# sarphiv/nerf-experiments

Measured on AMD Instinct MI355X. Metric: ray-samples/sec (coarse+fine), training step, higher is better.
Workload: dtype fp32

## Files before the change

### nerf-experiments_amd/csrc/mlp_fused.hip

```cpp
#include <stddef.h>
#include <stdlib.h>
#include <string.h>

#include <type_traits>

#include "common.h"
#include "encode_common.h"
#include "composite_common.h"
#include "hashgrid_common.h"

using namespace nerf;

typedef float f4 __attribute__((ext_vector_type(4)));
typedef float f8 __attribute__((ext_vector_type(8)));
typedef __bf16 bf16x8 __attribute__((ext_vector_type(8)));
typedef __bf16 bf16x4 __attribute__((ext_vector_type(4)));

namespace {

typedef __attribute__((address_space(3))) void lds_void_t;
typedef __attribute__((address_space(1))) void glb_void_t;

constexpr int SLOT_BYTES = 16 * 1024;
constexpr int NSLOT = 2;
// ... 223 lines not shown
template <int NS, class CT>
__device__ __forceinline__ void gen_hash_rows(const CT& c, int base, const float (&v)[9]) {
#pragma clang fp contract(off)
    float* R = reinterpret_cast<float*>(c.ximg);
    float* P = R + NS * GEN_LD;
    const int L = HG(int32_t, levels), F = HG(int32_t, features), T = HG(int32_t, table_size);
    const int cols = L * F;
    if (c.lane < NS) {
        float p[3] = {0.f, 0.f, 0.f};
        if (base + c.lane < c.M) {
            const float tq = HG(int32_t, query) == 0 ? v[6] : (v[6] + v[7]) / 2.0f;
            p[0] = v[0] + tq * v[3];
            p[1] = v[1] + tq * v[4];
            p[2] = v[2] + tq * v[5];
        }
        float* pr = P + c.lane * 8;
        pr[0] = p[0]; pr[1] = p[1]; pr[2] = p[2];
        float* row = R + c.lane * GEN_LD;
        for (int col = cols; col < 64; ++col) row[col] = 0.f;
    }
    const int normalize = HG(int32_t, normalize);
    const __attribute__((address_space(4))) int64_t* primes =
        (const __attribute__((address_space(4))) int64_t*)(c.kargs + offsetof(FusedArgs, hg) +
                                                           offsetof(nerf_hashgrid_params, primes));
    const long long pr[3] = {(long long)primes[0], (long long)primes[1], (long long)primes[2]};
    const __attribute__((address_space(4))) int32_t* res =
        (const __attribute__((address_space(4))) int32_t*)(c.kargs + offsetof(FusedArgs, hg) +
                                                           offsetof(nerf_hashgrid_params, res));
    const __attribute__((address_space(4))) int* offs =
        (const __attribute__((address_space(4))) int*)(c.kargs + offsetof(FusedArgs, hg_off));
    const float* table = *(const __attribute__((address_space(4))) cfptr_t*)(c.kargs + offsetof(FusedArgs, hg_table));
    for (int l = 0; l < L; ++l) {
        const int rl = res[l], ol = offs[l];
        if (c.lane < NS) {
            const int r = c.lane;
            const float p[3] = {P[r * 8 + 0], P[r * 8 + 1], P[r * 8 + 2]};
            const Corners cn = level_corners(p, normalize, rl, T, pr);
            const float* tab = table + (int64_t)ol * F;
            float* o = R + r * GEN_LD + l * F;
            float g[8][4];
#pragma unroll
            for (int k = 0; k < 8; ++k)
#pragma unroll
                for (int f = 0; f < 4; ++f) g[k][f] = f < F ? tab[(int64_t)cn.idx[k] * F + f] : 0.f;
            float acc[4] = {0.0f, 0.0f, 0.0f, 0.0f};
#pragma unroll
            for (int k = 0; k < 8; ++k)
#pragma unroll
                for (int f = 0; f < 4; ++f) acc[f] = acc[f] + cn.w[k] * g[k][f];
#pragma unroll
            for (int f = 0; f < 4; ++f)
                if (f < F) o[f] = acc[f];
        }
    }
}

template <int NS, class CT>
__device__ __forceinline__ void gen_rows_lds(const CT& c, int e, int base, const float (&v)[9]) {
#pragma clang fp contract(off)
    float* R = reinterpret_cast<float*>(c.ximg);
    float* P = R + NS * GEN_LD;
    const __attribute__((address_space(4))) nerf_pe_params& prm = EF(nerf_pe_params, params, e);
    if (prm.kind == 2) {
        gen_hash_rows<NS>(c, base, v);
        return;
    }
    const int per_ray = EF(int, per_ray, e);
    const int out_dim = EF(int, out_dim, e);
    const int L = prm.levels, id = prm.include_identity ? 3 : 0;
    if (c.lane < NS) {
        float pm[3] = {0.f, 0.f, 0.f}, vb[3] = {0.f, 0.f, 0.f};
        if (base + c.lane < c.M) {
            float p[3], dv[3];
            if (per_ray) {
                p[0] = v[0]; p[1] = v[1]; p[2] = v[2];
                dv[0] = dv[1] = dv[2] = 0.f;
            } else {
                const float tq = prm.query == 0 ? v[6] : (v[6] + v[7]) / 2.0f;
                dv[0] = v[3]; dv[1] = v[4]; dv[2] = v[5];
                p[0] = v[0] + tq * dv[0];
                p[1] = v[1] + tq * dv[1];
                p[2] = v[2] + tq * dv[2];
            }
            if (prm.kind == 1) {
                const IpeSample q = ipe_sample(prm, p, dv, v[6], v[7], v[8]);
                pm[0] = q.pm[0]; pm[1] = q.pm[1]; pm[2] = q.pm[2];
                vb[0] = q.vb[0]; vb[1] = q.vb[1]; vb[2] = q.vb[2];
            } else {
                pm[0] = p[0]; pm[1] = p[1]; pm[2] = p[2];
            }
        }
        float* pr = P + c.lane * 8;
        pr[0] = pm[0]; pr[1] = pm[1]; pr[2] = pm[2];
        pr[3] = vb[0]; pr[4] = vb[1]; pr[5] = vb[2];
        float* row = R + c.lane * GEN_LD;
        for (int col = 0; col < id; ++col) row[col] = pm[col];
        for (int col = out_dim; col < 64; ++col) row[col] = 0.f;
    }
    const int na = 3 * L;
    {
        static_assert(NS >= 16 && NS <= 64 && 64 % NS == 0, "mask lanes 0-15 in the g = 0 group");
        constexpr int G = 64 / NS;
        const int r = c.lane % NS, g = c.lane / NS;
        const float* pr = P + r * 8;
        const float pmr[3] = {pr[0], pr[1], pr[2]}, vbr[3] = {pr[3], pr[4], pr[5]};
        const float mreg = prm.use_mask ? prm.mask[c.lane & 15] : 1.f;
        const float scale = prm.scale;
        const int kind = prm.kind, use_mask = prm.use_mask;
        float* row = R + r * GEN_LD + id;
        for (int j = g; j < na; j += G) {
            const int dd = j >= 2 * L ? 2 : (j >= L ? 1 : 0);
            const int k = j - dd * L;
            const float sc = scale * (float)(1u << k);
            float sn, cs;
            sincos_enc(sel3(pmr, dd) * sc, &sn, &cs);
            if (kind == 1) {
                const float w = expf((-(sel3(vbr, dd) * (float)(1u << (2 * k)))) / 2.0f);
                cs = cs * w;
                sn = sn * w;
            }
            if (use_mask) {
                const float mk = __builtin_bit_cast(float, __builtin_amdgcn_ds_bpermute(k << 2, __builtin_bit_cast(int, mreg)));
                cs = mk * cs;
                sn = mk * sn;
            }
            row[j] = cs;
            row[na + j] = sn;
        }
    }
}

template <int NS, class CT>
__device__ __forceinline__ void gen_store(const CT& c, int e, int base) {
    const float* R = reinterpret_cast<const float*>(c.ximg);
    float* out = EF(fptr_t, out, e);
    const int per_ray = EF(int, per_ray, e);
    const unsigned S = (unsigned)EF(int, samples_per_ray, e);
    const int ld = (int)EF(int64_t, ld, e);
    const int q4 = ld >> 2;
    for (int i = c.lane; i < NS * q4; i += 64) {
        const int r = i / q4, q = i - r * q4;
        const int m = base + r;
        if (m < c.M && (!per_ray || (unsigned)m % S == 0u)) {
            const int64_t n = per_ray ? (int64_t)((unsigned)m / S) : (int64_t)m;
            *reinterpret_cast<f4*>(out + n * ld + 4 * q) = *reinterpret_cast<const f4*>(R + r * GEN_LD + 4 * q);
        }
    }
}

template <class CT>
__device__ __forceinline__ void gen_block(const CT& c, int r, int col, bf16x8& h, bf16x8& lo) {
    const float* R = reinterpret_cast<const float*>(c.ximg) + r * GEN_LD + col;
    const f4 v0 = *reinterpret_cast<const f4*>(R), v1 = *reinterpret_cast<const f4*>(R + 4);
    split8(__builtin_shufflevector(v0, v1, 0, 1, 2, 3, 4, 5, 6, 7), h, lo);
}

__device__ __forceinline__ void comp_grad_block(const Ctx& c, int gen, const float* coef, const int (&sample)[SB],
                                                const bool (&row_ok)[SB], bf16x8 (&h)[SB], bf16x8 (&lo)[SB]) {
#pragma clang fp contract(off)
    const unsigned S = (unsigned)CF(int32_t, samples_per_ray);
    const float* grgb = CF(cfptr_t, grad_rgb);
    const bool dens_head = CF(int32_t, sigma_layer) < 0;
    float* out = gen == 3 ? CF(fptr_t, grad_head) : CF(fptr_t, grad_sigma);
    const int64_t ldo = gen == 3 ? CF(int64_t, ld_head) : CF(int64_t, ld_sigma);
#pragma unroll
    for (int sb = 0; sb < SB; ++sb) {
        f4 x0 = {0.f, 0.f, 0.f, 0.f};
        if ((c.lane >> 4) == 0 && row_ok[sb]) {
            const unsigned m = (unsigned)sample[sb];
            const unsigned ray = m / S;
            const f4 q0 = *reinterpret_cast<const f4*>(coef + (size_t)m * 8);
            const f4 q1 = *reinterpret_cast<const f4*>(coef + (size_t)m * 8 + 4);
            const float g0 = grgb[ray * 3 + 0], g1 = grgb[ray * 3 + 1], g2 = grgb[ray * 3 + 2];
            const float ds = (g0 * q1[0] + g1 * q1[1]) + g2 * q1[2];
            if (gen == 3)
                x0 = f4{g0 * q0[0], g1 * q0[1], g2 * q0[2], dens_head ? ds : 0.f};
            else
                x0 = f4{ds, 0.f, 0.f, 0.f};
            if (out != nullptr) __builtin_nontemporal_store(x0, reinterpret_cast<f4*>(out + (size_t)m * ldo));
        }
        split8(__builtin_shufflevector(x0, f4{0.f, 0.f, 0.f, 0.f}, 0, 1, 2, 3, 4, 5, 6, 7), h[sb], lo[sb]);
    }
}

struct LayerState {
    int floor_i;
    bool qsplit;
    int col_chunk;
    int n1;
    unsigned bias_off;
    unsigned row_off[SB];
    unsigned row_off2[SB];
    int colok, colok2;
    unsigned sample_off[SB];
    unsigned mrow_off[SB];
    __amdgpu_buffer_rsrc_t ro, rm, rc, ro2;
    unsigned mw[SB][2];
    f4 stash[SB];
    unsigned pa[SB], pb[SB];
    unsigned pa2[SB], pb2[SB];
    int last_even;
    unsigned mi[SB][2];
    unsigned mcur[SB];
};

__device__ __forceinline__ void split2(float x, float y, unsigned& hi, unsigned& lo) {
    typedef __bf16 bf16x2 __attribute__((ext_vector_type(2)));
    typedef float f2 __attribute__((ext_vector_type(2)));
    const bf16x2 h = __builtin_convertvector((f4{x, y, 0.f, 0.f}).xy, bf16x2);
    hi = __builtin_bit_cast(unsigned, h);
    const f2 hf = {__builtin_bit_cast(float, hi << 16), __builtin_bit_cast(float, hi & 0xffff0000u)};
    const f2 d = f2{x, y} - hf;
    lo = __builtin_bit_cast(unsigned, __builtin_convertvector(d, bf16x2));
}

__device__ __forceinline__ unsigned hi2(float x, float y) {
    typedef __bf16 bf16x2 __attribute__((ext_vector_type(2)));
    return __builtin_bit_cast(unsigned, __builtin_convertvector((f4{x, y, 0.f, 0.f}).xy, bf16x2));
}

__device__ __forceinline__ bool pair_odd(int ch) { return ch >= 0 && (ch & 1) != 0; }

__device__ __forceinline__ float ror8(float x) {
    return __builtin_bit_cast(float, __builtin_amdgcn_mov_dpp(__builtin_bit_cast(int, x), 0x128, 0xf, 0xf, false));
}

__device__ __forceinline__ void pair_stores(const Ctx& c, const LayerState& st, int sb, int ch, int colok,
                                            unsigned pa, unsigned pb, const f4& y, f4& va, f4& vb, unsigned& oa,
                                            unsigned& ob) {
    const f4 x = st.stash[sb];
    const bool lo8 = (c.lane & 8) == 0;
    f4 rx, ry;
#pragma unroll
    for (int r = 0; r < 4; ++r) {
        const float xr = x[r], yr = y[r];
        rx[r] = ror8(xr);
        ry[r] = ror8(yr);
    }
    va = lo8 ? x : ry;
    vb = lo8 ? rx : y;
    const int cl = lo8 ? ch - 1 : ch;
    const bool inr = cl >= 0 && 16 * cl < colok;
    oa = inr ? pa + 64u * (unsigned)cl : OOB;
    ob = inr ? pb + 64u * (unsigned)cl : OOB;
}

template <int MODE, int EPAR = -1>
__device__ __forceinline__ void epi_part(Ctx& c, LayerState& st, int p, int ch, f4 (&a)[SB], f4 b) {
#ifdef NERF_FUSED_DIAG_NOEPI
    return;
#endif
#ifdef NERF_FUSED_DIAG_MFMAONLY
    if (p == 0) c.dsink += a[0][0] + a[0][3];
    return;
#endif
#ifdef NERF_FUSED_DIAG_NOMASK
    if (p == 2) return;
#endif
#ifdef NERF_FUSED_DIAG_NOSPLIT
    if (p == 3) return;
#endif
    const int q = ch >> 1, bb = ch & 1;
    if (p < 2) {
        if (p >= SB) return;
        const int sb = p;
        f4& v = a[sb];
        if constexpr (is_fwd(MODE)) {
#pragma unroll
            for (int r = 0; r < 4; ++r)
                v[r] = __builtin_bit_cast(float, max(__builtin_bit_cast(int, v[r] + b[r]), st.floor_i));
            if (ch >= 0 && ch == st.col_chunk) c.sig[sb] = v[0];
            f4 sv = v;
            if constexpr (is_qs(MODE)) {
                if (st.qsplit) {
                    typedef unsigned u2 __attribute__((ext_vector_type(2)));
                    typedef unsigned u4 __attribute__((ext_vector_type(4)));
                    unsigned h0, l0, h1, l1;
                    split2(v[0], v[1], h0, l0);
                    split2(v[2], v[3], h1, l1);
                    if (ch >= 0 && ch < 2 * KBMAX && ch < st.n1) {
                        char* d = c.ximg + ((q * SB + sb) * 2) * 1024 + c.lane * 16 + 8 * bb;
                        *reinterpret_cast<u2*>(d) = u2{h0, h1};
                        *reinterpret_cast<u2*>(d + 1024) = u2{l0, l1};
                    }
                    sv = __builtin_bit_cast(f4, u4{h0, h1, l0, l1});
                }
            }
            if (EPAR >= 0 ? EPAR == 0 : !pair_odd(ch)) {
                st.stash[sb] = sv;
                const unsigned off =
                    ch >= 0 && ch == st.last_even && 16 * ch < st.colok ? st.row_off[sb] + 64u * (unsigned)ch : OOB;
                __builtin_amdgcn_raw_buffer_store_b128(sv, st.ro, off, 0, ST_AUX);
                const unsigned coff = ch == st.col_chunk ? st.sample_off[sb] : OOB;
                __builtin_amdgcn_raw_buffer_store_b32(__builtin_bit_cast(unsigned, v[0]), st.rc, coff, 0, 0);
            } else {
                const unsigned oa = ch > 0 && 16 * (ch - 1) < st.colok ? st.row_off[sb] + 64u * (unsigned)(ch - 1) : OOB;
                const unsigned ob = ch >= 0 && 16 * ch < st.colok ? st.row_off[sb] + 64u * (unsigned)ch : OOB;
                __builtin_amdgcn_raw_buffer_store_b128(st.stash[sb], st.ro, oa, 0, ST_AUX);
                __builtin_amdgcn_raw_buffer_store_b128(sv, st.ro, ob, 0, ST_AUX);
            }
        } else {
            const bool sec = ch >= st.n1;
            const int sh = 4 * (7 - (ch & 7));
            if (ch == 8 && ch < st.n1) st.mcur[sb] = st.mi[sb][1];
            if (ch == st.n1) st.mcur[sb] = 0u;
#ifndef NERF_FUSED_DIAG_NOMASKIN
            if (ch >= 0) {
#pragma unroll
                for (int r = 0; r < 4; ++r) {
                    const int dead = __builtin_amdgcn_sbfe((int)st.mcur[sb], (unsigned)(sh + r), 1u);
                    const float x = v[r];
                    v[r] = __builtin_bit_cast(float, __builtin_bit_cast(int, x) & ~dead);
                }
            }
#else
            (void)sh;
#endif
#ifdef NERF_FUSED_DIAG_NOSTORE
            return;
#endif
#ifdef NERF_FUSED_DIAG_DROPSTORE
            st.colok = st.colok2 = -1 << 20;
            st.pa[sb] = st.pb[sb] = st.pa2[sb] = st.pb2[sb] = st.row_off[sb] = st.row_off2[sb] = OOB;
#endif
            if (EPAR >= 0 ? EPAR == 0 : !pair_odd(ch)) {
                st.stash[sb] = v;
                const bool alone = ch >= 0 && ch == st.last_even;
                const unsigned off1 = alone && !sec && 16 * ch < st.colok ? st.row_off[sb] + 64u * (unsigned)ch : OOB;
                const unsigned off2 =
                    alone && sec && 16 * (ch - st.n1) < st.colok2 ? st.row_off2[sb] + 64u * (unsigned)(ch - st.n1) : OOB;
                __builtin_amdgcn_raw_buffer_store_b128(v, st.ro, off1, 0, ST_AUX);
                __builtin_amdgcn_raw_buffer_store_b128(v, st.ro2, off2, 0, ST_AUX);
            } else if (!sec) {
                f4 va, vb;
                unsigned oa, ob;
                pair_stores(c, st, sb, ch, st.colok, st.pa[sb], st.pb[sb], v, va, vb, oa, ob);
                __builtin_amdgcn_raw_buffer_store_b128(va, st.ro, oa, 0, ST_AUX);
                __builtin_amdgcn_raw_buffer_store_b128(vb, st.ro, ob, 0, ST_AUX);
            } else {
                f4 va, vb;
                unsigned oa, ob;
                pair_stores(c, st, sb, ch - st.n1, st.colok2, st.pa2[sb], st.pb2[sb], v, va, vb, oa, ob);
                __builtin_amdgcn_raw_buffer_store_b128(va, st.ro2, oa, 0, ST_AUX);
                __builtin_amdgcn_raw_buffer_store_b128(vb, st.ro2, ob, 0, ST_AUX);
            }
        }
    } else if (p == 2) {
        if constexpr (is_fwd(MODE)) {
            if (ch >= 0 && ch < 2 * KBMAX) {
#pragma unroll
                for (int sb = 0; sb < SB; ++sb) {
                    unsigned t = st.mw[sb][1];
#pragma unroll
                    for (int r = 3; r >= 0; --r) t = shift_in_dead(t, a[sb][r]);
                    st.mw[sb][1] = t;
                }
                if (ch == 7) {
#pragma unroll
                    for (int sb = 0; sb < SB; ++sb) {
                        st.mw[sb][0] = st.mw[sb][1];
                        st.mw[sb][1] = 0;
                    }
                }
            }
        }
    } else {
        if (ch >= 0 && ch < 2 * KBMAX && ch < st.n1 && !(is_qs(MODE) && st.qsplit)) {
#pragma unroll
            for (int sb = 0; sb < SB; ++sb) {
                typedef unsigned u2 __attribute__((ext_vector_type(2)));
                char* d = c.ximg + ((q * SB + sb) * 2) * 1024 + c.lane * 16 + 8 * bb;
                if constexpr (is_x1(MODE)) {
                    *reinterpret_cast<u2*>(d) = u2{hi2(a[sb][0], a[sb][1]), hi2(a[sb][2], a[sb][3])};
                } else {
                    unsigned h0, l0, h1, l1;
                    split2(a[sb][0], a[sb][1], h0, l0);
                    split2(a[sb][2], a[sb][3], h1, l1);
                    const u2 h = {h0, h1}, lo = {l0, l1};
                    *reinterpret_cast<u2*>(d) = h;
                    *reinterpret_cast<u2*>(d + 1024) = lo;
                }
            }
        }
    }
}

template <int MODE, int EPAR>
__device__ __forceinline__ void epi_plain(Ctx& c, LayerState& st, int p, int ch, f4 (&a)[SB], f4 b) {
    static_assert(EPAR == 0 || EPAR == 1, "compile-time parity");
    const int q = ch >> 1;
    constexpr int bb = EPAR;
    if (p < 2) {
        if (p >= SB) return;
        const int sb = p;
        f4& v = a[sb];
        if constexpr (is_fwd(MODE)) {
#pragma unroll
            for (int r = 0; r < 4; ++r)
                v[r] = __builtin_bit_cast(float, max(__builtin_bit_cast(int, v[r] + b[r]), st.floor_i));
            f4 sv = v;
            if constexpr (is_qs(MODE)) {
                if (st.qsplit) {
                    typedef unsigned u2 __attribute__((ext_vector_type(2)));
                    typedef unsigned u4 __attribute__((ext_vector_type(4)));
                    unsigned h0, l0, h1, l1;
                    split2(v[0], v[1], h0, l0);
                    split2(v[2], v[3], h1, l1);
                    char* d = c.ximg + ((q * SB + sb) * 2) * 1024 + c.lane * 16 + 8 * bb;
                    *reinterpret_cast<u2*>(d) = u2{h0, h1};
                    *reinterpret_cast<u2*>(d + 1024) = u2{l0, l1};
                    sv = __builtin_bit_cast(f4, u4{h0, h1, l0, l1});
                }
            }
            if constexpr (EPAR == 0) {
                st.stash[sb] = sv;
            } else {
                const int so = 64 * (ch - 1);
                __builtin_amdgcn_raw_buffer_store_b128(st.stash[sb], st.ro, st.row_off[sb], so, ST_AUX);
                __builtin_amdgcn_raw_buffer_store_b128(sv, st.ro, st.row_off[sb] + 64u, so, ST_AUX);
            }
        } else {
            const int sh = 4 * (7 - (ch & 7));
            if constexpr (EPAR == 0) {
                if (ch == 8) st.mcur[sb] = st.mi[sb][1];
            }
#pragma unroll
            for (int r = 0; r < 4; ++r) {
                const int dead = __builtin_amdgcn_sbfe((int)st.mcur[sb], (unsigned)(sh + r), 1u);
                const float x = v[r];
                v[r] = __builtin_bit_cast(float, __builtin_bit_cast(int, x) & ~dead);
            }
            if constexpr (EPAR == 0) {
                st.stash[sb] = v;
            } else {
                const f4 x = st.stash[sb];
                const bool lo8 = (c.lane & 8) == 0;
                f4 rx, ry;
#pragma unroll
                for (int r = 0; r < 4; ++r) {
                    const float xr = x[r], yr = v[r];
                    rx[r] = ror8(xr);
                    ry[r] = ror8(yr);
                }
                const f4 va = lo8 ? x : ry;
                const f4 vb = lo8 ? rx : v;
                const int so = 64 * (ch - 1);
                __builtin_amdgcn_raw_buffer_store_b128(va, st.ro, st.pa[sb], so, ST_AUX);
                __builtin_amdgcn_raw_buffer_store_b128(vb, st.ro, st.pb[sb], so, ST_AUX);
            }
        }
    } else if (p == 2) {
        if constexpr (is_fwd(MODE)) {
#pragma unroll
            for (int sb = 0; sb < SB; ++sb) {
                unsigned t = st.mw[sb][1];
#pragma unroll
                for (int r = 3; r >= 0; --r) t = shift_in_dead(t, a[sb][r]);
                st.mw[sb][1] = t;
            }
            if constexpr (EPAR == 1) {
                if (ch == 7) {
#pragma unroll
                    for (int sb = 0; sb < SB; ++sb) {
                        st.mw[sb][0] = st.mw[sb][1];
                        st.mw[sb][1] = 0;
                    }
                }
            }
        }
    } else {
        if (!(is_qs(MODE) && st.qsplit)) {
#pragma unroll
            for (int sb = 0; sb < SB; ++sb) {
                typedef unsigned u2 __attribute__((ext_vector_type(2)));
                char* d = c.ximg + ((q * SB + sb) * 2) * 1024 + c.lane * 16 + 8 * bb;
                if constexpr (is_x1(MODE)) {
                    *reinterpret_cast<u2*>(d) = u2{hi2(a[sb][0], a[sb][1]), hi2(a[sb][2], a[sb][3])};
                } else {
                    unsigned h0, l0, h1, l1;
                    split2(a[sb][0], a[sb][1], h0, l0);
                    split2(a[sb][2], a[sb][3], h1, l1);
                    const u2 h = {h0, h1}, lo = {l0, l1};
                    *reinterpret_cast<u2*>(d) = h;
                    *reinterpret_cast<u2*>(d + 1024) = lo;
                }
            }
        }
    }
}

constexpr int EPI_NP = 3;
__host__ __device__ constexpr int epi_part_of(int i) {
    return i == 0 ? 0 : i + 1;
}
template <int KBR, int EPI0>
__host__ __device__ constexpr int epi_placed() {
    return KBR - EPI0 < EPI_NP ? (KBR - EPI0 > 0 ? KBR - EPI0 : 0) : EPI_NP;
}

template <int MODE>
constexpr int epi0_of() { return is_fwd(MODE) ? 3 : 4; }

constexpr int FA = 2;

template <int MODE, int KBR, int I>
__device__ __forceinline__ void first_reads(bf16x8 (&fr)[FA][2], unsigned sa) {
    if constexpr (I < FA && I < KBR) {
        lds_frag<I * 2048>(fr[I][0], sa);
        if constexpr (!is_x1(MODE)) lds_frag<I * 2048 + 1024>(fr[I][1], sa);
        first_reads<MODE, KBR, I + 1>(fr, sa);
    }
}

template <int MODE, int KBR, int KBH, int KB_I, int EPAR = -1, bool PL = false>
__device__ __forceinline__ void reg_steps(Ctx& c, LayerState& st, unsigned sa, bf16x8 (&fr)[FA][2], f4 (&a)[SB],
                                          f4 (&pv)[SB], f4& pb, int ch) {
    constexpr int EPI0 = KBR >= 8 ? epi0_of<MODE>() : (KBR >= 4 ? 1 : 0);
    if constexpr (KB_I < KBR) {
        bf16x8(&f)[2] = fr[KB_I % FA];
        constexpr int later = (KB_I + FA - 1 < KBR - 1 ? KB_I + FA - 1 : KBR - 1) - KB_I;
        if constexpr (is_x1(MODE)) {
            lds_wait1<later>(f[0]);
#pragma unroll
            for (int sb = 0; sb < SB; ++sb) a[sb] = mfma16(f[0], c.xh[KB_I][sb], a[sb]);
        } else {
            lds_wait<2 * later>(f[0], f[1]);
#pragma unroll
            for (int sb = 0; sb < SB; ++sb) a[sb] = mfma16(f[1], c.xh[KB_I][sb], a[sb]);
#pragma unroll
            for (int sb = 0; sb < SB; ++sb) a[sb] = mfma16(f[0], c.xl[KB_I][sb], a[sb]);
#pragma unroll
            for (int sb = 0; sb < SB; ++sb) a[sb] = mfma16(f[0], c.xh[KB_I][sb], a[sb]);
        }
        if constexpr (KB_I + FA < KBR) {
            lds_frag<(KB_I + FA) * 2048>(f[0], sa);
            if constexpr (!is_x1(MODE)) lds_frag<(KB_I + FA) * 2048 + 1024>(f[1], sa);
        }
        if constexpr (KB_I == EPI0 && is_fwd(MODE) && !(PL && EPAR == 2))
            bias_wait<(KBR > 0 ? DMA_PER_WAVE : 0) + (is_x1(MODE) ? 1 : 2) * KBH>(pb);
        if constexpr (KB_I >= EPI0 && KB_I < EPI0 + epi_placed<KBR, EPI0>()) {
            if constexpr (!PL)
                epi_part<MODE, EPAR>(c, st, epi_part_of(KB_I - EPI0), ch - 1, pv, pb);
            else if constexpr (EPAR != 2)
                epi_plain<MODE, EPAR>(c, st, epi_part_of(KB_I - EPI0), ch - 1, pv, pb);
        }
        __builtin_amdgcn_sched_barrier(0);
        reg_steps<MODE, KBR, KBH, KB_I + 1, EPAR, PL>(c, st, sa, fr, a, pv, pb, ch);
    }
}

template <int MODE, int KBR, int KBH>
__device__ __forceinline__ void fused_layer(Ctx& c, int l, int base) {
    constexpr int EPI0 = KBR >= 8 ? epi0_of<MODE>() : (KBR >= 4 ? 1 : 0);
    const int g = c.lane >> 4;
    const int N = LF(int, N, l);
    const int NC = n16_of(N);
    LayerState st;
    const int ldo = (int)LF(int64_t, ldo, l);
    st.floor_i = LF(int, relu, l) != 0 ? 0 : (int)0x80000000;
    st.qsplit = is_qs(MODE) &&
                ((*(const __attribute__((address_space(4))) int*)(c.kargs + offsetof(FusedArgs, split_mask)) >> l) & 1) != 0;
    st.colok = ldo - 4 * g;
    st.last_even = (NC & 1) ? NC - 1 : -1;
    int sample[SB];
    bool row_ok[SB];
#pragma unroll
    for (int sb = 0; sb < SB; ++sb) {
        sample[sb] = base + 16 * sb + (c.lane & 15);
        row_ok[sb] = sample[sb] < c.M;
        st.row_off[sb] = row_ok[sb] ? (unsigned)sample[sb] * (unsigned)ldo * 4u + 16u * g : OOB;
        st.sample_off[sb] = row_ok[sb] && g == 0 ? (unsigned)sample[sb] * 4u : OOB;
        st.mrow_off[sb] = row_ok[sb] ? (unsigned)sample[sb] * 32u + 8u * g : OOB;
        {
            const int sa = (c.lane & 8) == 0 ? sample[sb] : sample[sb] - 8;
            const int sbb = sa + 8;
            st.pa[sb] = sa < c.M ? (unsigned)sa * (unsigned)ldo * 4u + 16u * g : OOB;
            st.pb[sb] = sbb < c.M ? (unsigned)sbb * (unsigned)ldo * 4u + 16u * g : OOB;
        }
        st.mw[sb][0] = st.mw[sb][1] = 0;
    }
    st.ro = __builtin_amdgcn_make_buffer_rsrc(LF(fptr_t, out, l), 0, c.M * ldo * 4, RSRC_W3);
    st.bias_off = (unsigned)LF(int64_t, bias_off, l) + 16u * g;
    if constexpr (is_fwd(MODE)) {
        uint8_t* mptr = LF(u8ptr_t, mask, l);
        st.rm = __builtin_amdgcn_make_buffer_rsrc(mptr, 0, mptr != nullptr ? c.M * 32 : 0, RSRC_W3);
        float* cptr = LF(fptr_t, col_out, l);
        st.col_chunk = cptr != nullptr ? LF(int, col_idx, l) / 16 : -1;
        st.rc = __builtin_amdgcn_make_buffer_rsrc(cptr, 0, cptr ? c.M * 4 : 0, RSRC_W3);
        st.n1 = NC;
    } else {
        float* o2 = LF(fptr_t, out2, l);
        st.n1 = o2 != nullptr ? 2 * LF(int, n1, l) : NC;
        const int ldo2 = o2 != nullptr ? (int)LF(int64_t, ldo2, l) : 0;
        st.colok2 = ldo2 - 4 * g;
        st.ro2 = __builtin_amdgcn_make_buffer_rsrc(o2, 0, o2 ? c.M * ldo2 * 4 : 0, RSRC_W3);
#pragma unroll
        for (int sb = 0; sb < SB; ++sb)
            st.row_off2[sb] = row_ok[sb] ? (unsigned)sample[sb] * (unsigned)ldo2 * 4u + 16u * g : OOB;
#pragma unroll
        for (int sb = 0; sb < SB; ++sb) {
            const int sa = (c.lane & 8) == 0 ? sample[sb] : sample[sb] - 8;
            const int sbb = sa + 8;
            st.pa2[sb] = sa < c.M ? (unsigned)sa * (unsigned)ldo2 * 4u + 16u * g : OOB;
            st.pb2[sb] = sbb < c.M ? (unsigned)sbb * (unsigned)ldo2 * 4u + 16u * g : OOB;
        }
        const uint8_t* mi = LF(cu8ptr_t, mask_in, l);
        const __amdgpu_buffer_rsrc_t rmi =
            __builtin_amdgcn_make_buffer_rsrc(const_cast<uint8_t*>(mi), 0, mi != nullptr ? c.M * 32 : 0, RSRC_W3);
#pragma unroll
        for (int sb = 0; sb < SB; ++sb) {
            const unsigned off = st.mrow_off[sb];
            typedef unsigned u2 __attribute__((ext_vector_type(2)));
            const u2 w = __builtin_bit_cast(u2, __builtin_amdgcn_raw_buffer_load_b64(rmi, off, 0, 0));
            st.mi[sb][0] = w.x;
            st.mi[sb][1] = w.y;
            st.mcur[sb] = w.x;
        }
    }

    bool plain = false;
    if constexpr (KBR == 8 && KBH == 0) {
        plain = NERF_TU_BUILD_FLAGS == 0 &&
                *(const __attribute__((address_space(4))) int*)(c.kargs + offsetof(FusedArgs, no_plain)) == 0 &&
                (N & 31) == 0 && N <= 32 * KBMAX && ldo == N &&
                LF(fptr_t, out, l) != nullptr &&
                (is_fwd(MODE) ? LF(fptr_t, col_out, l) == nullptr : LF(fptr_t, out2, l) == nullptr);
        if constexpr (!is_fwd(MODE)) {
            if (plain) {
#pragma unroll
                for (int sb = 0; sb < SB; ++sb) {
                    const unsigned hi8 = (c.lane & 8) != 0 ? 64u : 0u;
                    st.pa[sb] += hi8;
                    st.pb[sb] += hi8;
                }
            }
        }
    }

    bf16x8 hh[KBH > 0 ? KBH : 1][SB], hl[KBH > 0 ? KBH : 1][SB];
    if constexpr (KBH > 0) {
        const int kb0 = LFI(int, seg_kb, 0, l);
#pragma unroll
        for (int kh = 0; kh < KBH; ++kh) {
            const int sg = kh < kb0 ? 0 : 1;
            const int khl = sg ? kh - kb0 : kh;
            const int gen = sg ? LFI(int, seg_gen, 1, l) : LFI(int, seg_gen, 0, l);
            if (!is_fwd(MODE) && gen >= 3) {
                comp_grad_block(c, gen, sg ? LFI(cfptr_t, seg_ptr, 1, l) : LFI(cfptr_t, seg_ptr, 0, l), sample,
                                row_ok, hh[kh], hl[kh]);
                continue;
            }
            if (is_fwd(MODE) && gen != 0) {
                if constexpr (KBR == 0) {
#pragma unroll
                    for (int sb = 0; sb < SB; ++sb)
                        gen_block(c, 16 * sb + (c.lane & 15), 32 * khl + 8 * g, hh[kh][sb], hl[kh][sb]);
                } else {
#pragma unroll
                    for (int sb = 0; sb < SB; ++sb) {
                        hh[kh][sb] = c.gh[sb];
                        hl[kh][sb] = c.gl[sb];
                    }
                }
                continue;
            }
            const float* p = sg ? LFI(cfptr_t, seg_ptr, 1, l) : LFI(cfptr_t, seg_ptr, 0, l);
            const int64_t ld = sg ? LFI(int64_t, seg_ld, 1, l) : LFI(int64_t, seg_ld, 0, l);
            const int k = sg ? LFI(int, seg_k, 1, l) : LFI(int, seg_k, 0, l);
            const int rd = sg ? LFI(int, seg_rd, 1, l) : LFI(int, seg_rd, 0, l);
            const int rows = sg ? LFI(int, seg_rows, 1, l) : LFI(int, seg_rows, 0, l);
            const __amdgpu_buffer_rsrc_t rs =
                __builtin_amdgcn_make_buffer_rsrc(const_cast<float*>(p), 0, (int)((int64_t)rows * ld * 4), RSRC_W3);
            const int col = 32 * khl + 8 * g;
#pragma unroll
            for (int sb = 0; sb < SB; ++sb) {
                const unsigned m = (unsigned)(row_ok[sb] ? sample[sb] : 0);
                const unsigned row = rd == 1 ? m : m / (unsigned)rd;
                const unsigned rbase = (unsigned)(((int64_t)row * ld + col) * 4);
                const f4 x0 = __builtin_amdgcn_raw_buffer_load_b128(rs, col < k ? rbase : OOB, 0, 0);
                const f4 x1 = __builtin_amdgcn_raw_buffer_load_b128(rs, col + 4 < k ? rbase + 16 : OOB, 0, 0);
                split8(__builtin_shufflevector(x0, x1, 0, 1, 2, 3, 4, 5, 6, 7), hh[kh][sb], hl[kh][sb]);
            }
        }
    }
    if constexpr (KBH > 0) {
#pragma unroll
        for (int kh = 0; kh < KBH; ++kh)
#pragma unroll
            for (int sb = 0; sb < SB; ++sb) {
                if constexpr (is_x1(MODE))
                    asm volatile("" : "+v"(hh[kh][sb]));
                else
                    asm volatile("" : "+v"(hh[kh][sb]), "+v"(hl[kh][sb]));
            }
    }
    const unsigned hbm_frag = (unsigned)LF(int, hbm_off, l) + (unsigned)c.lane * 16u;

    f4 pv[SB] = {};
    auto last_epilogue = [&](auto pl_tag) __attribute__((always_inline)) {
        f4 lb = {0.f, 0.f, 0.f, 0.f};
        if constexpr (is_fwd(MODE)) {
            buf_load16(lb, st.bias_off + 64u * (unsigned)(NC - 1), c.rimg);
            bias_wait<0>(lb);
        }
#pragma unroll
        for (int p = 0; p < 4; ++p) {
            if constexpr (decltype(pl_tag)::value)
                epi_plain<MODE, 1>(c, st, p, NC - 1, pv, lb);
            else
                epi_part<MODE>(c, st, p, NC - 1, pv, lb);
        }
    };
    if constexpr (KBR == 0) {
        typedef bf16x8 fragk_t[KBH > 0 ? KBH : 1][2];
        auto frag_load = [&](fragk_t& f, int ch) __attribute__((always_inline)) {
#pragma unroll
            for (int kh = 0; kh < KBH; ++kh)
#pragma unroll
                for (int hl_ = 0; hl_ < (is_x1(MODE) ? 1 : 2); ++hl_)
                    f[kh][hl_] = __builtin_bit_cast(
                        bf16x8, __builtin_amdgcn_raw_buffer_load_b128(
                                    c.rimg, hbm_frag + (unsigned)(((ch * KBH + kh) * 2 + hl_) * 1024), 0, 0));
        };
        auto bias_load = [&](int ch) __attribute__((always_inline)) {
            return __builtin_bit_cast(f4, __builtin_amdgcn_raw_buffer_load_b128(
                                              c.rimg, st.bias_off + (is_fwd(MODE) ? 64u * (unsigned)ch : 0u), 0, 0));
        };
        fragk_t hA, hB;
        f4 bA, bB = f4{0.f, 0.f, 0.f, 0.f};
        frag_load(hA, 0);
        auto step = [&](int ch, fragk_t& cur, fragk_t& nxt, f4& bthis, const f4& bprev) __attribute__((always_inline)) {
            frag_load(nxt, ch + 1 < NC ? ch + 1 : ch);
            bthis = bias_load(ch);
            f4 a[SB];
#pragma unroll
            for (int sb = 0; sb < SB; ++sb) a[sb] = f4{0.f, 0.f, 0.f, 0.f};
#pragma unroll
            for (int kh = 0; kh < KBH; ++kh) {
                if constexpr (!is_x1(MODE)) {
#pragma unroll
                    for (int sb = 0; sb < SB; ++sb) a[sb] = mfma16(cur[kh][1], hh[kh][sb], a[sb]);
#pragma unroll
                    for (int sb = 0; sb < SB; ++sb) a[sb] = mfma16(cur[kh][0], hl[kh][sb], a[sb]);
                }
#pragma unroll
                for (int sb = 0; sb < SB; ++sb) a[sb] = mfma16(cur[kh][0], hh[kh][sb], a[sb]);
            }
#pragma unroll
            for (int i = 0; i < EPI_NP; ++i) epi_part<MODE>(c, st, epi_part_of(i), ch - 1, pv, bprev);
#pragma unroll
            for (int sb = 0; sb < SB; ++sb) pv[sb] = a[sb];
        };
        for (int ch = 0; ch < NC; ch += 2) {
            step(ch, hA, hB, bA, bB);
            if (ch + 1 < NC) step(ch + 1, hB, hA, bB, bA);
        }
        last_epilogue(std::false_type{});
    } else
    {
    auto chunk = [&](int ch, auto ep_tag, auto vm_tag) __attribute__((always_inline)) {
        constexpr int EP = decltype(ep_tag)::value;
        constexpr int VM = decltype(vm_tag)::value;
        constexpr bool PL = VM >= 0;
        static_assert(!PL || (KBR == 8 && KBH == 0), "plain layers: register-fed only");
        f4 pb = {0.f, 0.f, 0.f, 0.f};
        if constexpr (is_fwd(MODE) && !(PL && EP == 2))
            buf_load16(pb, st.bias_off + 64u * (unsigned)(PL || ch > 0 ? ch - 1 : 0), c.rimg);
        const unsigned sa = lds_addr(c.smem + c.cur * SLOT_BYTES + c.lane * 16);
        bf16x8 fr[FA][2];
        if constexpr (KBR > 0) {
            asm volatile("s_waitcnt vmcnt(%0)" ::"n"(PL ? VM : after_dma_vm<MODE>()) : "memory");
#ifndef NERF_FUSED_DIAG_NOBARRIER
            barrier();
#endif
#ifdef NERF_FUSED_DIAG_BAR2
            barrier();
#endif
            first_reads<MODE, KBR, 0>(fr, sa);
            issue_dma(c, c.cur ^ 1);
            __builtin_amdgcn_sched_barrier(0);
        }
        bf16x8 hf[KBH > 0 ? KBH : 1][2];
#pragma unroll
        for (int kh = 0; kh < KBH; ++kh)
#pragma unroll
            for (int hl_ = 0; hl_ < (is_x1(MODE) ? 1 : 2); ++hl_)
                buf_load16(hf[kh][hl_], hbm_frag + (unsigned)(((ch * KBH + kh) * 2 + hl_) * 1024), c.rimg);
        f4 a[SB];
#pragma unroll
        for (int sb = 0; sb < SB; ++sb) a[sb] = f4{0.f, 0.f, 0.f, 0.f};
        reg_steps<MODE, KBR, KBH, 0, EP, PL>(c, st, sa, fr, a, pv, pb, ch);
#pragma unroll
        for (int kh = 0; kh < KBH; ++kh) {
            if constexpr (is_x1(MODE))
                frag_vwait1<(KBR > 0 ? 2 * SB : 0)>(hf[kh][0]);
            else
                frag_vwait<(KBR > 0 ? 2 * SB : 0)>(hf[kh][0], hf[kh][1]);
        }
#pragma unroll
        for (int kh = 0; kh < KBH; ++kh) {
            if constexpr (!is_x1(MODE)) {
#pragma unroll
                for (int sb = 0; sb < SB; ++sb) a[sb] = mfma16(hf[kh][1], hh[kh][sb], a[sb]);
#pragma unroll
                for (int sb = 0; sb < SB; ++sb) a[sb] = mfma16(hf[kh][0], hl[kh][sb], a[sb]);
            }
#pragma unroll
            for (int sb = 0; sb < SB; ++sb) a[sb] = mfma16(hf[kh][0], hh[kh][sb], a[sb]);
            __builtin_amdgcn_sched_barrier(0);
        }
        if constexpr (KBR == 0) bias_wait<0>(pb);
#pragma unroll
        for (int i = epi_placed<KBR, EPI0>(); i < EPI_NP; ++i) {
            if constexpr (!PL) epi_part<MODE, EP>(c, st, epi_part_of(i), ch - 1, pv, pb);
        }
        if constexpr (KBR > 0) c.cur ^= 1;
#pragma unroll
        for (int sb = 0; sb < SB; ++sb) pv[sb] = a[sb];
    };
    auto generic_loop = [&]() __attribute__((always_inline)) {
        for (int ch = 0; ch < NC; ch += 2) {
            chunk(ch, std::integral_constant<int, 1>{}, std::integral_constant<int, -1>{});
            if (ch + 1 < NC) chunk(ch + 1, std::integral_constant<int, 0>{}, std::integral_constant<int, -1>{});
        }
        last_epilogue(std::false_type{});
    };
    if constexpr (KBR == 8 && KBH == 0) {
        if (plain) {
            constexpr int V_LO = is_fwd(MODE) ? 1 : 0, V_HI = is_fwd(MODE) ? 3 : 2;
            chunk(0, std::integral_constant<int, 2>{}, std::integral_constant<int, V_HI>{});
            chunk(1, std::integral_constant<int, 0>{}, std::integral_constant<int, V_LO>{});
            for (int ch = 2; ch < NC; ch += 2) {
                chunk(ch, std::integral_constant<int, 1>{}, std::integral_constant<int, V_LO>{});
                chunk(ch + 1, std::integral_constant<int, 0>{}, std::integral_constant<int, V_HI>{});
            }
            last_epilogue(std::true_type{});
        } else {
            generic_loop();
        }
    } else {
        generic_loop();
    }
    }
    if constexpr (is_fwd(MODE)) {
        const int nb = NC < 2 * KBMAX ? NC : 2 * KBMAX;
        if (nb < 8) {
#pragma unroll
            for (int sb = 0; sb < SB; ++sb) {
                st.mw[sb][0] = st.mw[sb][1] << (4 * (8 - nb));
                st.mw[sb][1] = 0;
            }
        } else if (nb > 8) {
#pragma unroll
            for (int sb = 0; sb < SB; ++sb) st.mw[sb][1] <<= 4 * (16 - nb);
        }
        typedef unsigned u2 __attribute__((ext_vector_type(2)));
#pragma unroll
        for (int sb = 0; sb < SB; ++sb)
            __builtin_amdgcn_raw_buffer_store_b64(u2{st.mw[sb][0], st.mw[sb][1]}, st.rm, st.mrow_off[sb], 0, 0);
    }
    if constexpr (is_fwd(MODE)) {
#pragma unroll
        for (int sb = 0; sb < SB; ++sb) c.head[sb] = pv[sb];
    }
    if (l + 1 == c.n_layers) return;
#pragma unroll
    for (int kb = 0; kb < KBMAX; ++kb)
#pragma unroll
        for (int sb = 0; sb < SB; ++sb) {
            c.xh[kb][sb] = *reinterpret_cast<const bf16x8*>(c.ximg + ((kb * SB + sb) * 2) * 1024 + c.lane * 16);
            c.xl[kb][sb] = *reinterpret_cast<const bf16x8*>(c.ximg + ((kb * SB + sb) * 2 + 1) * 1024 + c.lane * 16);
        }
}

constexpr int COMP_OFF = 8192;
constexpr int COMP_SMAX = 2 * TILE;
constexpr int COMP_DEL = COMP_SMAX * 16;
static_assert(COMP_OFF >= SB * 2048 && COMP_OFF + COMP_SMAX * 20 <= XIMG_BYTES, "composite scratch");

template <int R, class CT>
__device__ __forceinline__ void composite_wave(CT& c, int64_t ray, int S, int roff = 0) {
    const char* reg = c.ximg + COMP_OFF + roff;
    float rd[R], del[R], rc[R][3];
#pragma unroll
    for (int r = 0; r < R; ++r) {
        const int s = r * 64 + c.lane;
        rd[r] = 0.f; del[r] = 0.f;
        rc[r][0] = rc[r][1] = rc[r][2] = 0.f;
        if (s < S) {
            const f4 h = *reinterpret_cast<const f4*>(reg + s * 16);
            rc[r][0] = h[0]; rc[r][1] = h[1]; rc[r][2] = h[2]; rd[r] = h[3];
            del[r] = *reinterpret_cast<const float*>(reg + COMP_DEL + s * 4);
        }
    }
    float w[R], rgb[3], cc[R][3], cs[R][3];
    composite_ray<R, true>(S, CF(float, scale_a), CF(float, scale_b), 1, CF(float, density_shift), c.lane, rd, del,
                           rc, w, rgb, cc, cs);
    const int64_t base = ray * S;
    float* wo = CF(fptr_t, weights);
    float* co = CF(fptr_t, coef);
#pragma unroll
    for (int r = 0; r < R; ++r) {
        const int s = r * 64 + c.lane;
        if (s < S) {
            if (wo != nullptr) __builtin_nontemporal_store(w[r], wo + base + s);
            if (co != nullptr) {
                f4* q = reinterpret_cast<f4*>(co + (base + s) * 8);
                __builtin_nontemporal_store(f4{cc[r][0], cc[r][1], cc[r][2], 0.f}, q);
                __builtin_nontemporal_store(f4{cs[r][0], cs[r][1], cs[r][2], 0.f}, q + 1);
            }
        }
    }
    if (c.lane == 0) {
        float* o = CF(fptr_t, rgb) + ray * 3;
        __builtin_nontemporal_store(rgb[0], o);
        __builtin_nontemporal_store(rgb[1], o + 1);
        __builtin_nontemporal_store(rgb[2], o + 2);
    }
}

__device__ __forceinline__ void composite_tile(Ctx& c, int tile) {
#ifdef NERF_FUSED_DIAG_NOCOMP
    return;
#endif
    const int S = CF(int32_t, samples_per_ray);
    const bool col_sigma = CF(int32_t, sigma_layer) >= 0;
    if (S > TILE) {
        if ((tile & 1) == 0) {
#pragma unroll
            for (int sb = 0; sb < SB; ++sb) {
                c.phead[sb] = c.head[sb];
                if (col_sigma) c.phead[sb][3] = c.sig[sb];
                c.pcdist[sb] = c.cdist[sb];
            }
            return;
        }
        if (c.lane < 16) {
            char* reg = c.smem + NSLOT * SLOT_BYTES + COMP_OFF;
#pragma unroll
            for (int sb = 0; sb < SB; ++sb) {
                const int j = c.wave * SPW + 16 * sb + c.lane;
                f4 h = c.head[sb];
                if (col_sigma) h[3] = c.sig[sb];
                *reinterpret_cast<f4*>(reg + j * 16) = c.phead[sb];
                *reinterpret_cast<float*>(reg + COMP_DEL + j * 4) = c.pcdist[sb];
                *reinterpret_cast<f4*>(reg + (TILE + j) * 16) = h;
                *reinterpret_cast<float*>(reg + COMP_DEL + (TILE + j) * 4) = c.cdist[sb];
            }
        }
        barrier();
        asm volatile("" ::: "memory");
        if (c.wave == 0) composite_wave<(2 * TILE) / 64>(c, (int64_t)(tile >> 1), S);
        return;
    }
    if (c.lane < 16) {
#pragma unroll
        for (int sb = 0; sb < SB; ++sb) {
            const int j = c.wave * SPW + 16 * sb + c.lane;
            if (tile * TILE + j < c.M) {
                const int r = j / S, o = j - r * S;
                char* reg = c.smem + NSLOT * SLOT_BYTES + r * XIMG_BYTES + COMP_OFF;
                f4 h = c.head[sb];
                if (col_sigma) h[3] = c.sig[sb];
                *reinterpret_cast<f4*>(reg + o * 16) = h;
                *reinterpret_cast<float*>(reg + COMP_DEL + o * 4) = c.cdist[sb];
            }
        }
    }
    barrier();
    asm volatile("" ::: "memory");
    const int rpt = TILE / S;
    const int64_t ray = (int64_t)tile * rpt + c.wave;
    if (c.wave < rpt && ray * S < c.M) {
        if (S > 64)
            composite_wave<2>(c, ray, S);
        else
            composite_wave<1>(c, ray, S);
    }
}

template <int MODE>
__global__ __launch_bounds__(WG) __attribute__((amdgpu_waves_per_eu(NWAVE / 4, NWAVE / 4))) void mlp_fused_kernel(FusedArgs a) {
    __shared__ __attribute__((aligned(16))) char smem[NSLOT * SLOT_BYTES + NWAVE * XIMG_BYTES];
    Ctx c;
    c.kargs = (kchar_t*)__builtin_amdgcn_kernarg_segment_ptr();
    c.smem = smem;
    c.rimg = __builtin_amdgcn_make_buffer_rsrc(const_cast<char*>(a.img), 0, a.img_bytes, RSRC_W3);
    c.wave = __builtin_amdgcn_readfirstlane(threadIdx.x >> 6);
    c.ximg = smem + NSLOT * SLOT_BYTES + c.wave * XIMG_BYTES;
    c.lane = threadIdx.x & 63;
    c.M = a.M;
    c.n_layers = a.n_layers;
    c.dsink = 0.f;
    if ((int)blockIdx.x >= a.ntiles) return;
    const int ngroups = a.ntiles / a.span;
    const int my_tiles = a.span * ((ngroups - (int)blockIdx.x + (int)gridDim.x - 1) / (int)gridDim.x);
    int per_tile = 0;
    for (int l = 0; l < a.n_layers; ++l)
        if (dma_units(c, l) > 0) per_tile += n16_of(LF(int, N, l));
    c.d_remaining = my_tiles * per_tile;
    {
        const int l = c.lane < c.n_layers ? c.lane : 0;
        c.t_off = (int)LF(int64_t, img_off, l);
        c.t_units = dma_units(c, l);
        c.t_n16 = n16_of(LF(int, N, l));
        c.t_next = next_ring_layer(c, l + 1 == c.n_layers ? 0 : l + 1);
    }
    const int l0 = next_ring_layer(c, 0);
    if (l0 >= 0) dma_seek(c, l0);
    c.cur = 0;
    if (l0 >= 0) issue_dma(c, 0);
    asm volatile("s_waitcnt vmcnt(0)" ::: "memory");
    __syncthreads();
#pragma unroll
    for (int kb = 0; kb < KBMAX; ++kb)
#pragma unroll
        for (int sb = 0; sb < SB; ++sb) {
            c.xh[kb][sb] = bf16x8{};
            c.xl[kb][sb] = bf16x8{};
        }
#pragma unroll
    for (int sb = 0; sb < SB; ++sb) {
        c.gh[sb] = bf16x8{};
        c.gl[sb] = bf16x8{};
    }
    const int span_log = a.span >> 1;
    auto tile_of = [&](int it) { return (((int)blockIdx.x + (it >> span_log) * (int)gridDim.x) << span_log) + (it & span_log); };
    float gv0[9], gv1[9];
    if (is_fwd(MODE) && a.gen_mask != 0 && my_tiles > 0) {
        const int nb = tile_of(0) * TILE + c.wave * SPW;
        if (a.gen_mask & 1) gen_load<SPW>(c, 0, nb, gv0);
        if (a.gen_mask & 2) gen_load<SPW>(c, 1, nb, gv1);
    }
    for (int it = 0; it < my_tiles; ++it) {
        const int tile = tile_of(it);
        const int base = tile * TILE + c.wave * SPW;
        if (is_fwd(MODE) && a.comp_on) {
            const float* dist = CF(cfptr_t, dist);
#pragma unroll
            for (int sb = 0; sb < SB; ++sb) {
                const int m = base + 16 * sb + (c.lane & 15);
                c.cdist[sb] = c.lane < 16 && m < c.M ? dist[m] : 0.f;
            }
        }
#ifndef NERF_FUSED_DIAG_NOGEN
        if (is_fwd(MODE) && a.gen_mask != 0) {
#else
        if (false) {
#endif
            float v0[9], v1[9];
#pragma unroll
            for (int j = 0; j < 9; ++j) {
                v0[j] = gv0[j];
                v1[j] = gv1[j];
            }
#ifdef NERF_FUSED_DIAG_GEN2
#pragma nounroll
            for (int i = 0; i < 4; ++i) {
                const int e = a.gen_lds == 0 ? 1 - (i & 1) : (i & 1);
#else
#pragma nounroll
            for (int i = 0; i < 2; ++i) {
                const int e = a.gen_lds == 0 ? 1 - i : i;
#endif
                if ((a.gen_mask >> e) & 1) {
                    float v[9];
#pragma unroll
                    for (int j = 0; j < 9; ++j) v[j] = e == 0 ? v0[j] : v1[j];
                    gen_rows_lds<SPW>(c, e, base, v);
                    if (e == a.gen_reg) {
#pragma unroll
                        for (int sb = 0; sb < SB; ++sb)
                            gen_block(c, 16 * sb + (c.lane & 15), 8 * (c.lane >> 4), c.gh[sb], c.gl[sb]);
                    }
                    gen_store<SPW>(c, e, base);
                }
            }
        }
        for (int l = 0; l < a.n_layers; ++l) {
            if (is_fwd(MODE) && a.gen_mask != 0 && it + 1 < my_tiles &&
                l == (a.n_layers > 2 ? a.n_layers - 2 : 0)) {
                const int nb = tile_of(it + 1) * TILE + c.wave * SPW;
                if (a.gen_mask & 1) gen_load<SPW>(c, 0, nb, gv0);
                if (a.gen_mask & 2) gen_load<SPW>(c, 1, nb, gv1);
            }
            switch (LF(int, type, l)) {
                case 1: fused_layer<MODE, 0, 1>(c, l, base); break;
                case 2: fused_layer<MODE, 0, 2>(c, l, base); break;
                case 3: fused_layer<MODE, 4, 0>(c, l, base); break;
                case 6: fused_layer<MODE, 8, 0>(c, l, base); break;
                case 7: fused_layer<MODE, 8, 1>(c, l, base); break;
                case 8: fused_layer<MODE, 8, 2>(c, l, base); break;
                default: break;
            }
        }
        if (is_fwd(MODE) && a.comp_on) composite_tile(c, tile);
#ifdef NERF_FUSED_DIAG_COMP2
        if (is_fwd(MODE) && a.comp_on) composite_tile(c, tile);
#endif
    }
#ifdef NERF_FUSED_DIAG_MFMAONLY
    if (c.dsink == 1234.5f) LF(fptr_t, out, 0)[threadIdx.x] = c.dsink;
#endif
}
#undef LF
#undef LFI
#undef EF
#undef CF
#undef HG

struct PackArgs {
    const float* src[NERF_FUSED_MAX_SRCS];
};

__global__ __launch_bounds__(256) void fused_pack_kernel(PackArgs p, const int32_t* __restrict__ map_src,
                                                         const int32_t* __restrict__ map_dst, int64_t n,
                                                         char* __restrict__ img) {
    const int64_t i = (int64_t)blockIdx.x * 256 + threadIdx.x;
    if (i >= n) return;
    const int s = map_src[i];
    float v = 0.f;
    if (s >= 0) {
        typedef __attribute__((address_space(4))) const float* const kptr_t;
        kptr_t* tab = (kptr_t*)((kchar_t*)__builtin_amdgcn_kernarg_segment_ptr() + offsetof(PackArgs, src));
        v = tab[s >> 24][s & 0xffffff];
    }
    const int d = map_dst[i];
    if (d >= 0) {
        const __bf16 hi = (__bf16)v;
        const __bf16 lo = (__bf16)(v - (float)hi);
        __bf16* b = reinterpret_cast<__bf16*>(img);
        b[d] = hi;
        b[d + 512] = lo;
    } else {
        reinterpret_cast<float*>(img)[~d] = v;
    }
}

int num_cus() {
    static int n = 0;
    if (n == 0) {
        int dev = 0;
        if (hipGetDevice(&dev) != hipSuccess ||
            hipDeviceGetAttribute(&n, hipDeviceAttributeMultiprocessorCount, dev) != hipSuccess || n <= 0)
            n = 256;
    }
    return n;
}

}

namespace {
int enc_out_dim(const nerf_pe_params& p) { return (2 * p.levels + (p.include_identity ? 1 : 0)) * 3; }

bool hash_ok(const nerf_fused_encoding& e) {
    const nerf_hashgrid_params* h = e.hash;
    if (h == nullptr || e.hash_table == nullptr || !aligned16(e.hash_table)) return false;
    if (h->levels < 1 || h->levels > 16 || !(h->features == 1 || h->features == 2 || h->features == 4)) return false;
    if (h->table_size < 1 || (int64_t)h->levels * h->table_size * h->features >= ((int64_t)1 << 31)) return false;
    if (!(h->normalize == 0 || h->normalize == 1) || !(h->query == 0 || h->query == 1)) return false;
    if (e.params.query != h->query || e.per_ray || e.out_dim != h->levels * h->features) return false;
    for (int l = 0; l < h->levels; ++l)
        if (h->res[l] < 1 || h->res[l] > (1 << 20)) return false;
    return true;
}

bool encoding_ok(const nerf_fused_encoding& e, int64_t M) {
    const nerf_pe_params& p = e.params;
// ... 248 lines not shown
```

Before: 72.45 million.

## Defer backward mask-row load into loop branches and reuse prefetched last-layer bias

Moves the backward-pass mask row load out of the common setup so that for the KBR==8 path it is issued inside the plain and generic loop branches, closer to use, with a retire hook keeping the values live. The KBR==0 path now hands its already-loaded bias register to the last epilogue instead of reloading and waiting on it. Mask-switch updates are skipped for odd-parity epilogue calls. It also drops the early return for the last layer, so the final x-image reload now always runs, which adds some LDS reads.

New measurement: 72.99 million (median of 6 runs). Within noise of the previous version (+0.8%).

```diff
diff --git a/nerf-experiments_amd/csrc/mlp_fused.hip b/nerf-experiments_amd/csrc/mlp_fused.hip
--- a/nerf-experiments_amd/csrc/mlp_fused.hip
+++ b/nerf-experiments_amd/csrc/mlp_fused.hip
@@ -549,8 +549,10 @@
         } else {
             const bool sec = ch >= st.n1;
             const int sh = 4 * (7 - (ch & 7));
-            if (ch == 8 && ch < st.n1) st.mcur[sb] = st.mi[sb][1];
-            if (ch == st.n1) st.mcur[sb] = 0u;
+            if constexpr (EPAR != 1) {
+                if (ch == 8 && ch < st.n1) st.mcur[sb] = st.mi[sb][1];
+                if (ch == st.n1) st.mcur[sb] = 0u;
+            }
 #ifndef NERF_FUSED_DIAG_NOMASKIN
             if (ch >= 0) {
 #pragma unroll
@@ -851,19 +853,30 @@
             st.pa2[sb] = sa < c.M ? (unsigned)sa * (unsigned)ldo2 * 4u + 16u * g : OOB;
             st.pb2[sb] = sbb < c.M ? (unsigned)sbb * (unsigned)ldo2 * 4u + 16u * g : OOB;
         }
-        const uint8_t* mi = LF(cu8ptr_t, mask_in, l);
-        const __amdgpu_buffer_rsrc_t rmi =
-            __builtin_amdgcn_make_buffer_rsrc(const_cast<uint8_t*>(mi), 0, mi != nullptr ? c.M * 32 : 0, RSRC_W3);
-#pragma unroll
-        for (int sb = 0; sb < SB; ++sb) {
-            const unsigned off = st.mrow_off[sb];
-            typedef unsigned u2 __attribute__((ext_vector_type(2)));
-            const u2 w = __builtin_bit_cast(u2, __builtin_amdgcn_raw_buffer_load_b64(rmi, off, 0, 0));
-            st.mi[sb][0] = w.x;
-            st.mi[sb][1] = w.y;
-            st.mcur[sb] = w.x;
-        }
-    }
+    }
+    auto mask_load = [&]() __attribute__((always_inline)) {
+        if constexpr (!is_fwd(MODE)) {
+            const uint8_t* mi = LF(cu8ptr_t, mask_in, l);
+            const __amdgpu_buffer_rsrc_t rmi =
+                __builtin_amdgcn_make_buffer_rsrc(const_cast<uint8_t*>(mi), 0, mi != nullptr ? c.M * 32 : 0, RSRC_W3);
+#pragma unroll
+            for (int sb = 0; sb < SB; ++sb) {
+                const unsigned off = st.mrow_off[sb];
+                typedef unsigned u2 __attribute__((ext_vector_type(2)));
+                const u2 w = __builtin_bit_cast(u2, __builtin_amdgcn_raw_buffer_load_b64(rmi, off, 0, 0));
+                st.mi[sb][0] = w.x;
+                st.mi[sb][1] = w.y;
+                st.mcur[sb] = w.x;
+            }
+        }
+    };
+    if constexpr (!(KBR == 8 && KBH == 0)) mask_load();
+    auto mask_retire = [&]() __attribute__((always_inline)) {
+        if constexpr (!is_fwd(MODE)) {
+#pragma unroll
+            for (int sb = 0; sb < SB; ++sb) asm volatile("" ::"v"(st.mi[sb][1]));
+        }
+    };
 
     bool plain = false;
     if constexpr (KBR == 8 && KBH == 0) {
@@ -944,11 +957,15 @@
     const unsigned hbm_frag = (unsigned)LF(int, hbm_off, l) + (unsigned)c.lane * 16u;
 
     f4 pv[SB] = {};
-    auto last_epilogue = [&](auto pl_tag) __attribute__((always_inline)) {
+    auto last_epilogue = [&](auto pl_tag, const f4* have) __attribute__((always_inline)) {
         f4 lb = {0.f, 0.f, 0.f, 0.f};
         if constexpr (is_fwd(MODE)) {
-            buf_load16(lb, st.bias_off + 64u * (unsigned)(NC - 1), c.rimg);
-            bias_wait<0>(lb);
+            if (have != nullptr) {
+                lb = *have;
+            } else {
+                buf_load16(lb, st.bias_off + 64u * (unsigned)(NC - 1), c.rimg);
+                bias_wait<0>(lb);
+            }
         }
 #pragma unroll
         for (int p = 0; p < 4; ++p) {
@@ -998,11 +1015,15 @@
 #pragma unroll
             for (int sb = 0; sb < SB; ++sb) pv[sb] = a[sb];
         };
-        for (int ch = 0; ch < NC; ch += 2) {
+        int ch = 0;
+        do {
             step(ch, hA, hB, bA, bB);
             if (ch + 1 < NC) step(ch + 1, hB, hA, bB, bA);
-        }
-        last_epilogue(std::false_type{});
+        } while ((ch += 2) < NC);
+        const f4 lbias = (NC & 1) ? bA : bB;
+        if constexpr (!is_fwd(MODE)) asm volatile("" ::"v"(lbias));
+        mask_retire();
+        last_epilogue(std::false_type{}, &lbias);
     } else
     {
     auto chunk = [&](int ch, auto ep_tag, auto vm_tag) __attribute__((always_inline)) {
@@ -1070,19 +1091,25 @@
             chunk(ch, std::integral_constant<int, 1>{}, std::integral_constant<int, -1>{});
             if (ch + 1 < NC) chunk(ch + 1, std::integral_constant<int, 0>{}, std::integral_constant<int, -1>{});
         }
-        last_epilogue(std::false_type{});
+        mask_retire();
+        last_epilogue(std::false_type{}, nullptr);
     };
     if constexpr (KBR == 8 && KBH == 0) {
         if (plain) {
             constexpr int V_LO = is_fwd(MODE) ? 1 : 0, V_HI = is_fwd(MODE) ? 3 : 2;
+            if constexpr (!is_fwd(MODE)) asm volatile("; plain loop: mask row");
+            mask_load();
             chunk(0, std::integral_constant<int, 2>{}, std::integral_constant<int, V_HI>{});
             chunk(1, std::integral_constant<int, 0>{}, std::integral_constant<int, V_LO>{});
             for (int ch = 2; ch < NC; ch += 2) {
                 chunk(ch, std::integral_constant<int, 1>{}, std::integral_constant<int, V_LO>{});
                 chunk(ch + 1, std::integral_constant<int, 0>{}, std::integral_constant<int, V_HI>{});
             }
-            last_epilogue(std::true_type{});
+            mask_retire();
+            last_epilogue(std::true_type{}, nullptr);
         } else {
+            if constexpr (!is_fwd(MODE)) asm volatile("; generic loop: mask row");
+            mask_load();
             generic_loop();
         }
     } else {
@@ -1110,7 +1137,6 @@
 #pragma unroll
         for (int sb = 0; sb < SB; ++sb) c.head[sb] = pv[sb];
     }
-    if (l + 1 == c.n_layers) return;
 #pragma unroll
     for (int kb = 0; kb < KBMAX; ++kb)
 #pragma unroll
```
